# kenziyuliu/ChineseCheckersAgent

Measured on AMD Instinct MI355X. Metric: mcts_node_expansions_per_s (self-play with the policy/value net, 4096 games x 400 sims/move per GPU); BASELINE games/s = config.games_per_s: selfplay() calls that RETURNED per second, discarded ones included (train.py:61-64 counts them); config.games_won_per_s: those that returned a history, higher is better.
Workload: dtype f32

## Files before the change

### chinesecheckersagent_amd/csrc/ccsp_net.hip

```cpp
#include <cmath>
#include <cstring>
#include <type_traits>
#include <vector>
#include "ccsp_common.h"

namespace {

typedef float f32x4 __attribute__((ext_vector_type(4)));

#ifndef CCSP_NET_LDX
#define CCSP_NET_LDX 68
#define CCSP_NET_LDY 36
#endif
constexpr int LDX = CCSP_NET_LDX;
constexpr int LDY = CCSP_NET_LDY;
constexpr int LDI = 12;
constexpr int NPOL = 294, NPOL_PAD = 304;
#ifndef CCSP_NET_LDS_BIAS_ALL
#define CCSP_NET_LDS_BIAS_ALL 0
#endif
#ifndef CCSP_NET_PDG
#define CCSP_NET_PDG 1
#endif
#ifndef CCSP_NET_SEG_STEM
// ... 473 lines not shown
                  NW = C::NW, F32 = C::F32, F32A = C::F32A, F64 = C::F64, F64B = C::F64B, M64 = C::M64, XT = C::XT, HB = C::HB;
    constexpr bool AS = C::ALLSPLIT;
    extern __shared__ __attribute__((aligned(16))) unsigned char smem_raw[];
    Smem<C> &S = *reinterpret_cast<Smem<C> *>(smem_raw);
    const int tid = threadIdx.x, lane = tid & 63;
    const int wave = __builtin_amdgcn_readfirstlane(tid >> 6);
    const int q = lane >> 4, l15 = lane & 15;
    const long long s0 = (long long)blockIdx.x * NB;
    const int here = (int)((n - s0) < NB ? (n - s0) : NB);

    WBuf wb;
    wb.r = __builtin_amdgcn_make_buffer_rsrc(const_cast<float *>(W), 0, LAY.total * 4, 0x00020000);
    wb.voff = lane * 16;

#ifdef CCSP_STAMPS
    if (blockIdx.x == 0 && threadIdx.x == 0) net_stamps[62] = __builtin_amdgcn_s_memtime();
#endif
    float *in = S.y2;
    static_assert((PADROWS * LDY) % 4 == 0, "y1 is cleared 16 bytes at a time");
    for (int i = tid * 4; i < PADROWS * LDY; i += NTH * 4) *reinterpret_cast<f32x4 *>(&S.y1[i]) = f32x4{0.f, 0.f, 0.f, 0.f};
    if constexpr (NB < 8 || CCSP_NET_LDS_BIAS_ALL)
    for (int i = tid; i < BIAS_N / 4; i += NTH)
        *reinterpret_cast<f32x4 *>(&S.bias[4 * i]) = *reinterpret_cast<const f32x4 *>(W + LAY.trunk_b + 4 * i);
    const ccsp_request *rq = reinterpret_cast<const ccsp_request *>(planes) + s0;
    if constexpr (REQ) {
        static_assert((INROWS * LDI) % 4 == 0, "the staging area is cleared 16 bytes at a time");
        for (int i = tid * 4; i < INROWS * LDI; i += NTH * 4) *reinterpret_cast<f32x4 *>(&in[i]) = f32x4{0.f, 0.f, 0.f, 0.f};
        __syncthreads();
        struct PlaneWriter {
            float *base;
            struct Ref { float *p; __device__ __forceinline__ void operator=(uint8_t val) const { *p = (float)val; } };
            __device__ __forceinline__ Ref operator[](int i) const { const int cell = i / 7; return Ref{base + cell * LDI + (i - 7 * cell)}; }
        };
        for (int t = tid; t < here * 12; t += NTH) {
            const int s = t / 12, k = t - 12 * s;
            if (rq[s].kind == 0) continue;
            const ccsp_sr st = ccsp_load_sr(&rq[s].state);
            ccsp_scatter_checker(st, (int)rq[s].player, k, PlaneWriter{in + s * 49 * LDI});
        }
        for (int t = tid; t < here * 49; t += NTH) {
            const int s = t / 49, cell = t - 49 * s;
            if (rq[s].kind != 0 && rq[s].player == 2) in[(s * 49 + cell) * LDI + 6] = 1.0f;
        }
    } else if constexpr ((NB * 343) % 4 != 0) {
        for (int i = tid; i < INROWS * LDI; i += NTH) {
            const int cellg = i / LDI, ch = i % LDI, s = cellg / 49, cell = cellg % 49;
            in[i] = (ch < 7 && s < here) ? planes[(s0 + s) * 343 + cell * 7 + ch] : 0.0f;
        }
    } else {
        constexpr int NV = (NB * 343) / 4, PER = (NV + NTH - 1) / NTH;
        const f32x4 *src = reinterpret_cast<const f32x4 *>(planes + s0 * 343);
        const int nreal = here * 343;
        f32x4 v[PER];
#pragma unroll
        for (int r = 0; r < PER; r++) {
            const int e = (tid + r * NTH) * 4;
            v[r] = f32x4{0.f, 0.f, 0.f, 0.f};
            if (e + 3 < nreal) v[r] = src[tid + r * NTH];
            else if (e < nreal) { for (int j = 0; j < 4; j++) if (e + j < nreal) v[r][j] = planes[s0 * 343 + e + j]; }
        }
        static_assert((INROWS * LDI) % 4 == 0, "the staging area is cleared 16 bytes at a time");
        for (int i = tid * 4; i < INROWS * LDI; i += NTH * 4) *reinterpret_cast<f32x4 *>(&in[i]) = f32x4{0.f, 0.f, 0.f, 0.f};
        __syncthreads();
#pragma unroll
        for (int r = 0; r < PER; r++) {
            const int e = (tid + r * NTH) * 4;
#pragma unroll
            for (int j = 0; j < 4; j++) {
                const unsigned ee = (unsigned)(e + j);
                if ((int)ee < nreal) {
                    const unsigned cellg = __umulhi(ee, 613566757u);
                    in[cellg * LDI + (ee - 7u * cellg)] = v[r][j];
                }
            }
        }
    }
#ifdef CCSP_EXP_NET_INPUT_DELAY
    __builtin_amdgcn_s_sleep(CCSP_EXP_NET_INPUT_DELAY);
#endif
    __syncthreads();
    NET_STAMP(0);
#ifdef CCSP_STAMPS
    if (blockIdx.x == 0 && threadIdx.x == 0) net_stamps[60] = __builtin_amdgcn_s_memrealtime();
#endif

    const int nt2 = wave & 1, qr = wave >> 1, mt3 = AS ? qr % MT : F32 * qr;
    const int kshare = XT ? (C::CELLMAJOR ? (qr == 0 ? C::xseg_of(0) : (qr == 1 ? C::xseg_of(1) : (qr == 2 ? C::xseg_of(2) : C::xseg_of(3)))) : qr) : -1;
    const int kh = AS ? qr / MT : 0;
    f32x4 pre[NPREMAX];
    constexpr bool CM = C::CELLMAJOR;
    auto row_sp = [&](int row, int &s, int &pos) {
        if constexpr (CM) { const int t = row >> 4, l = row & 15; pos = cell_of<NB>(t < MT - 1 ? t * (16 / NB) + l / NB : 24); s = l % NB; }
        else { if (row >= ROWS) row -= 25; s = row / 25; pos = row % 25; }
    };
    auto y1_at = [&](int s, int pos, bool top_left) -> int {
        if constexpr (CM) return ((6 * (pos / 5) + pos % 5 + CM_PAD - (top_left ? 7 : 0)) * NB + s) * LDY + 4 * q;
        else return ((top_left ? 0 : PAD0) + s * PADPOS + (pos / 5) * 6 + (pos % 5)) * LDY + 4 * q;
    };
    constexpr int TAPROW = (CM ? NB : 1) * LDY;
    constexpr bool LDS_BIAS = NB < 8 || CCSP_NET_LDS_BIAS_ALL;
    auto bias4 = [&](int idx) -> f32x4 {
        if constexpr (LDS_BIAS) return *reinterpret_cast<const f32x4 *>(&S.bias[idx + 4 * q]);
        else return *reinterpret_cast<const f32x4 *>(W + LAY.trunk_b + idx + 4 * q);
    };
    auto relu4 = [](const f32x4 &v) -> f32x4 { return f32x4{relu(v[0]), relu(v[1]), relu(v[2]), relu(v[3])}; };

    f32x4 xr[F64];
    lds_float *const xown = lds_opaque(&S.x[(((wave >> 2) * M64) * 16 + l15) * LDX + (wave & 3) * 16 + 4 * q]);
    {
        const int nt = wave & 3, mt0 = (wave >> 2) * M64;
        int sbase[F64];
#pragma unroll
        for (int i = 0; i < F64; i++) {
            const int row = (mt0 + i) * 16 + l15;
            int s = row / 25, pos = row % 25;
            if constexpr (CM) row_sp(row, s, pos);
            sbase[i] = (s * 49 + (pos / 5) * 7 + (pos % 5)) * LDI + (q & 1) * 4;
        }
        int tapoff[5];
#pragma unroll
        for (int kb = 0; kb < 5; kb++) {
            const int tap = kb * 2 + (q >> 1);
            tapoff[kb] = ((tap / 3) * 7 + tap % 3) * LDI;
        }
        auto afrag = [&](int, int kb, int i) -> f32x4 {
            return *reinterpret_cast<const f32x4 *>(&in[sbase[i] + tapoff[kb]]);
        };
        const f32x4 bv = bias4(BIAS_STEM + nt * 16);
        auto epi = [&](int, const f32x4 &acc, int i) {
            xr[i] = relu4(acc + bv);
            lds_store4(xown, i * 16 * LDX, xr[i]);
        };
        prefetch<5>(wb, LAY.stem_w, nt, pre);
        auto next = [&]() { prefetch<4>(wb, LAY.l1_w[0], nt2, pre); };
        if (F64B == F64 || (wave >> 2) == 0) gemm_tiles<F64, 5, CCSP_NET_SEG_STEM>(wb, LAY.stem_w, nt, mt0, pre, afrag, next, epi);
        else gemm_tiles<F64B, 5, CCSP_NET_SEG_STEM>(wb, LAY.stem_w, nt, mt0, pre, afrag, next, epi);
    }
    __syncthreads();
    NET_STAMP(1);

    const lds_float *y1p[F32A + 1];
    bool prow_ok[F32A];
#pragma unroll
    for (int i = 0; i < F32A + 1; i++) {
        int s, pos;
        row_sp((i < F32A ? mt3 + i : MT - 1) * 16 + l15, s, pos);
        y1p[i] = lds_opaque(&S.y1[y1_at(s, pos, true)]);
        if (i < F32A) prow_ok[i] = (mt3 + i) * 16 + l15 < ROWS;
    }
    constexpr int CELL0 = 7 * TAPROW;
    const lds_float *const xin = lds_opaque(&S.x[(mt3 * 16 + l15) * LDX + 4 * q]);
    const lds_float *const xinx = lds_opaque(&S.x[((MT - 1) * 16 + l15) * LDX + 4 * q]);
    lds_float *const y2w = lds_opaque(&S.y2[(mt3 * 16 + l15) * LDY + nt2 * 16 + 4 * q]);
    const lds_float *const y2r = lds_opaque(&S.y2[(((wave >> 2) * M64) * 16 + l15) * LDY + 4 * q]);
    lds_float *const partw = lds_opaque(&S.part[AS ? mt3 * 2 + nt2 : nt2][(AS ? kh : (XT ? kshare : 0)) * (C::NSEG / C::NSH)][lane * 4]);
    const lds_float *const partr = lds_opaque(&S.part[AS ? ((wave >> 2) * M64) * 2 : 0][0][lane * 4]);
    constexpr bool TAIL4 = NB == 8 && CM && XT == 1 && CCSP_NET_TAIL_4X4 != 0;
    static_assert(!TAIL4 || (C::NSEG == 4 && NSPLIT == 4), "one segment job on each of the waves 0 .. 3");
    const int trow = 4 * ((lane >> 2) & 1) + (lane & 3), tcol = 4 * (lane >> 3) + (lane & 3);
    WBuf wbt = wb;
    wbt.voff = ((tcol >> 4) * 18 * 256 + (tcol & 15) * 4) * 4;
    const lds_float *ytail = nullptr;
    lds_float *partt = nullptr;
    if constexpr (TAIL4) {
        constexpr int pos = CELL8[24];
        ytail = lds_opaque(&S.y1[((6 * (pos / 5) + pos % 5 + CM_PAD - 7) * NB + trow) * LDY]);
        partt = lds_opaque(&S.part[tcol >> 4][0][(16 * ((tcol >> 2) & 3) + 4 * ((lane >> 2) & 1)) * 4 + (tcol & 3)]);
    }

    f32x4 bq2[AS ? 18 / C::NSH : 1];
    for (int blk = 0; blk < 9; blk++) {
        const int wo = blk * BLK_STRIDE, bb = BIAS_BLK + blk * BIAS_PER_BLK;
        int n2o = nt2 * 16;
        asm volatile("" : "+s"(n2o));
        {
            auto afrag = [&](int, int kb, int i) -> f32x4 {
                return i < F32A ? lds_load4(xin, i * 16 * LDX + kb * 16) : lds_load4(xinx, kb * 16);
            };
            const f32x4 bv = bias4(bb + BIAS_L1 + nt2 * 16);
            auto epi = [&](int, const f32x4 &acc, int i) {
                const lds_float *at = i == 0 ? y1p[0] : (i == 1 ? y1p[F32A > 1 ? 1 : 0] : y1p[F32A > 2 ? 2 : 0]);
                if constexpr (C::PADFULL) {
                    if (!(i == 0 ? prow_ok[0] : (i == 1 ? prow_ok[F32A > 1 ? 1 : 0] : prow_ok[F32A > 2 ? 2 : 0]))) return;
                }
                lds_store4(const_cast<lds_float *>(at), CELL0 + n2o, relu4(acc + bv));
            };
            auto epix = [&](const f32x4 &acc) {
                if (l15 < ROWS - (MT - 1) * 16) lds_store4(const_cast<lds_float *>(y1p[F32A]), CELL0 + n2o, relu4(acc + bv));
            };
            if constexpr (AS) ksplit_load<18, C::NSH>(wb, (LAY.l2_w[0] + wo), nt2, kh, bq2);
            if constexpr (AS) {
                auto epi1 = [&](int, const f32x4 &acc, int) {
                    if (prow_ok[0]) lds_store4(const_cast<lds_float *>(y1p[0]), CELL0 + n2o, relu4(acc + bv));
                };
                if (kh == 0) gemm_tiles<1, 4, CCSP_NET_SEG_L1>(wb, (LAY.l1_w[0] + wo), nt2, mt3, pre, afrag, []() {}, epi1);
            } else
            {
                auto next = [&]() { prefetch<18>(wb, (LAY.l2_w[0] + wo), nt2, pre); };
                if constexpr (CM && NB < 8) {
                    if (kshare == NSPLIT - 1) gemm_tiles_last<F32A, 4, NSPLIT, CCSP_NET_SEG_L1, 1>(wb, (LAY.l1_w[0] + wo), nt2, mt3, MT - 1, kshare, pre, afrag, next, epi, epix);
                    else gemm_tiles_last<F32A, 4, NSPLIT, CCSP_NET_SEG_L1, 0>(wb, (LAY.l1_w[0] + wo), nt2, mt3, MT - 1, kshare, pre, afrag, next, epi, epix);
                } else
                    gemm_tiles_last<F32A, 4, NSPLIT, CCSP_NET_SEG_L1, -1>(wb, (LAY.l1_w[0] + wo), nt2, mt3, MT - 1, kshare, pre, afrag, next, epi, epix);
            }
        }
        __syncthreads();
        NET_STAMP(2 + 3 * blk);
        {
            auto afrag = [&](int, int kb, int i) -> f32x4 {
                const int tap = kb >> 1;
                return lds_load4(y1p[i], ((tap / 3) * 6 + tap % 3) * TAPROW + (kb & 1) * 16);
            };
            const f32x4 bv = bias4(bb + BIAS_L2 + nt2 * 16);
            auto epi = [&](int, const f32x4 &acc, int i) { lds_store4(y2w, i * 16 * LDY, relu4(acc + bv)); };
            if constexpr (AS) {
                auto afrag_rt = [&](int kb) -> f32x4 {
                    const int tap = kb >> 1;
                    return lds_load4(y1p[0], ((tap / 3) * 6 + tap % 3) * TAPROW + (kb & 1) * 16);
                };
                gemm_ksplit<18, C::NSEG, C::NSH>(bq2, kh, afrag_rt, partw);
                prefetch<2>(wb, (LAY.l3_w[0] + wo), wave & 3, pre);
            } else
            {
                auto next = [&]() { prefetch<2>(wb, (LAY.l3_w[0] + wo), wave & 3, pre); };
                if constexpr (CM) {
                    auto run = [&](auto G) {
                        constexpr int g = decltype(G)::value;
                        if constexpr (TAIL4) {
                            gemm_tiles_split<F32A, 18, C::NSEG, NSPLIT, C::NE, true, C::dead_of(g, 0), C::dead_of(g, 1), -1>(wb, (LAY.l2_w[0] + wo), nt2, mt3, MT - 1, 0, pre, afrag, next, epi, partw);
                            if constexpr (g < 2) {
                                auto afrag4 = [&](int kb, int q4) -> f32x4 {
                                    const int tap = kb >> 1;
                                    return lds_load4(ytail, ((tap / 3) * 6 + tap % 3) * TAPROW + (kb & 1) * 16 + 4 * q4);
                                };
                                auto job = [&](auto SEG) {
                                    constexpr int seg = decltype(SEG)::value, kb0 = (18 * seg) / C::NSEG, kb1 = (18 * (seg + 1)) / C::NSEG;
                                    const f32x4 t = tail_tile_4x4<kb0, kb1 - kb0>(wbt, (LAY.l2_w[0] + wo), afrag4);
#pragma unroll
                                    for (int r = 0; r < 4; r++) partt[seg * 256 + r * 4] = t[r];
                                };
                                if (nt2 == 0) job(std::integral_constant<int, 2 * g>{});
                                else job(std::integral_constant<int, 2 * g + 1>{});
                            }
                        } else
                        gemm_tiles_split<F32A, 18, C::NSEG, NSPLIT, C::NE, true, C::dead_of(g, 0), C::dead_of(g, 1), C::xseg_of(g)>(wb, (LAY.l2_w[0] + wo), nt2, mt3, MT - 1, 0, pre, afrag, next, epi, partw);
                    };
                    if (qr == 0) run(std::integral_constant<int, 0>{});
                    else if (NSPLIT == 2 || qr == 1) run(std::integral_constant<int, 1>{});
                    else if (qr == 2) run(std::integral_constant<int, NSPLIT == 2 ? 1 : 2>{});
                    else run(std::integral_constant<int, NSPLIT == 2 ? 1 : 3>{});
                } else
                    gemm_tiles_split<F32A, 18, C::NSEG, NSPLIT, 0, false, 0u, 0u, 0>(wb, (LAY.l2_w[0] + wo), nt2, mt3, MT - 1, kshare, pre, afrag, next, epi, partw);
            }
            NET_STAMP(32 + blk);
#ifdef CCSP_STAMPS
            if (blockIdx.x == 0 && lane == 0 && blk == 4) {
                net_stamps[44 + wave] = __builtin_amdgcn_s_memtime();
                net_stamps[52 + wave] = __builtin_amdgcn_s_getreg(4 | (0 << 6) | (31 << 11));
            }
#endif
        }
        __syncthreads();
        NET_STAMP(3 + 3 * blk);
        {
            const int nt = wave & 3, half = wave >> 2, mt0 = half * M64;
            NET_STAMP2(0);
            const bool has_x = AS || (XT && half == C::NH - 1);
            constexpr int XSLOT = F64B - 1;
            const int xt = AS ? mt0 : 0;
            f32x4 ax[2];
            if (has_x) {
#pragma unroll
                for (int kb = 0; kb < 2; kb++) {
                    f32x4 v = lds_load4(partr, kb * C::NSEG * 256);
#pragma unroll
                    for (int c = 1; c < C::NSEG; c++) v = v + lds_load4(partr, (kb * C::NSEG + c) * 256);
                    ax[kb] = relu4(v + bias4(bb + BIAS_L2 + kb * 16));
                }
            }
            auto afrag = [&](int mt, int kb, int i) -> f32x4 {
                if (i == XSLOT && has_x) return ax[kb];
                return lds_load4(y2r, i * 16 * LDY + kb * 16);
            };
            const f32x4 bv = bias4(bb + BIAS_L3 + nt * 16);
            auto epi = [&](int mt, const f32x4 &acc, int i) {
                xr[i] = relu4(acc + bv + xr[i]);
                lds_store4(xown, i * 16 * LDX, xr[i]);
            };
            NET_STAMP2(1);
            auto next = [&]() {
                NET_STAMP2(2);
                prefetch<4>(wb, blk < 8 ? LAY.l1_w[0] + wo + BLK_STRIDE : LAY.pc_w, blk < 8 ? nt2 : 0, pre);
            };
            if (F64B == F64 || half == 0) gemm_tiles<F64, 2, CCSP_NET_SEG_L3>(wb, (LAY.l3_w[0] + wo), nt, mt0, pre, afrag, next, epi);
            else gemm_tiles<F64B, 2, CCSP_NET_SEG_L3>(wb, (LAY.l3_w[0] + wo), nt, mt0, pre, afrag, next, epi);
            NET_STAMP2(3);
        }
        __syncthreads();
        NET_STAMP2(4);
        NET_STAMP(4 + 3 * blk);
    }

    float *pc = S.y1;
    {
        const int mt0 = 2 * wave < MT - 2 ? 2 * wave : MT - 2;
        const lds_float *const xpc = lds_opaque(&S.x[(mt0 * 16 + l15) * LDX + 4 * q]);
        auto afrag = [&](int, int kb, int i) -> f32x4 { return lds_load4(xpc, i * 16 * LDX + kb * 16); };
        const f32x4 bv = bias4(BIAS_PC);
        int pcat[2];
#pragma unroll
        for (int i = 0; i < 2; i++) {
            const int row = (mt0 + i) * 16 + l15;
            int s, pos;
            row_sp(row, s, pos);
            pcat[i] = (CM ? (row < ROWS ? s * 25 + pos : row) : row) * 16 + 4 * q;
        }
        auto epi = [&](int, const f32x4 &acc, int i) {
            *reinterpret_cast<f32x4 *>(&pc[pcat[i]]) = relu4(acc + bv);
        };
        gemm_tiles<2, 4, CCSP_NET_SEG_PC>(wb, LAY.pc_w, 0, mt0, pre, afrag, []() {}, epi);
    }
    float *vc = S.y2;
    float *lg = S.y2 + 256;
    if (tid < ROWS) {
        const float *wv = W + LAY.vc_w;
        float acc = W[LAY.vc_b];
        const float *xr = &S.x[tid * LDX];
#pragma unroll 8
        for (int k = 0; k < 64; k++) acc += xr[k] * wv[k];
        int s, pos;
        row_sp(tid, s, pos);
        vc[CM ? s * 25 + pos : tid] = acc > 0.f ? acc : 0.f;
    }
    __syncthreads();
    NET_STAMP(29);

    float *part = S.x;
    {
        constexpr int GPQ = 25, NHALF = NW / 4, TPW = (5 + NHALF - 1) / NHALF, PG = HB / 4, PDG = C::PDG;
        const int kq = wave & 3, th = wave >> 2;
        int woff[TPW];
        bool valid[TPW];
#pragma unroll
        for (int t = 0; t < TPW; t++) {
            const int T = th * TPW + t;
            valid[t] = T < 5;
            woff[t] = LAY.pf_w + ((valid[t] ? T : 0) * 100 + kq * GPQ) * 256;
        }
        f32x4 acc[TPW][PG], bq[PDG + 1][TPW];
#pragma unroll
        for (int t = 0; t < TPW; t++)
#pragma unroll
            for (int g = 0; g < PG; g++) acc[t][g] = f32x4{0.f, 0.f, 0.f, 0.f};
#pragma unroll
        for (int d = 0; d < PDG; d++)
#pragma unroll
            for (int t = 0; t < TPW; t++) bq[d][t] = wb.load(woff[t] + d * 256);
        const float *arow = &pc[(lane & 3) * 400 + kq * GPQ * 4];
        f32x4 a[2][PG];
#pragma unroll
        for (int g = 0; g < PG; g++) a[0][g] = *reinterpret_cast<const f32x4 *>(arow + g * 1600);
#pragma unroll
        for (int kg = 0; kg < GPQ; kg++) {
            if (kg + 1 < GPQ) {
#pragma unroll
                for (int g = 0; g < PG; g++) a[(kg + 1) & 1][g] = *reinterpret_cast<const f32x4 *>(arow + g * 1600 + (kg + 1) * 4);
            }
            if (kg + PDG < GPQ) {
#pragma unroll
                for (int t = 0; t < TPW; t++) bq[(kg + PDG) % (PDG + 1)][t] = wb.load(woff[t] + (kg + PDG) * 256);
            }
#pragma unroll
            for (int t = 0; t < TPW; t++) {
                if (t + 1 < TPW || valid[t]) {
#pragma unroll
                    for (int j = 0; j < 4; j++)
#pragma unroll
                        for (int g = 0; g < PG; g++)
                            acc[t][g] = __builtin_amdgcn_mfma_f32_4x4x1f32(a[kg & 1][g][j], bq[kg % (PDG + 1)][t][j], acc[t][g], 0, 0, 0);
                }
            }
        }
#pragma unroll
        for (int t = 0; t < TPW; t++) {
            if (valid[t]) {
                const int T = th * TPW + t;
#pragma unroll
                for (int g = 0; g < PG; g++)
#pragma unroll
                    for (int r = 0; r < 4; r++) part[(kq * HB + 4 * g + r) * 320 + T * 64 + lane] = acc[t][g][r];
            }
        }
    }
    __syncthreads();
    for (int i = tid; i < NB * NPOL; i += NTH) {
        const int s = i / NPOL, col = i - s * NPOL;
        const float q0 = part[(0 * HB + s) * 320 + col], q1 = part[(1 * HB + s) * 320 + col], q2 = part[(2 * HB + s) * 320 + col],
                    q3 = part[(3 * HB + s) * 320 + col];
        lg[s * NPOL_PAD + col] = ((q0 + q1) + q2) + q3 + W[LAY.pf_b + col];
    }
    float *h1 = S.y2 + 256 + NB * NPOL_PAD;
    if (tid < NB * 32) {
        const int s = tid >> 5, u = tid & 31;
        const float *w1 = W + LAY.f1_w;
        float acc = W[LAY.f1_b + u];
#pragma unroll 5
        for (int i = 0; i < 25; i++) acc += vc[s * 25 + i] * w1[i * 32 + u];
        h1[s * 32 + u] = acc > 0.f ? acc : 0.f;
    }
    __syncthreads();
    NET_STAMP(30);
    if (tid < here) {
        const float *w2 = W + LAY.f2_w;
        float acc = W[LAY.f2_b];
        for (int u = 0; u < 32; u++) acc += h1[tid * 32 + u] * w2[u];
        if (!REQ || rq[tid].kind != 0) v_out[s0 + tid] = tanhf(acc);
    }
    for (int s = wave; s < here; s += NTH / 64) {
        const float *row = lg + s * NPOL_PAD;
        float mx = -INFINITY;
        for (int i = lane; i < NPOL; i += 64) mx = fmaxf(mx, row[i]);
        for (int m = 32; m >= 1; m >>= 1) mx = fmaxf(mx, __shfl_xor(mx, m));
        double e[5];
        double sum = 0.0;
#pragma unroll
        for (int j = 0; j < 5; j++) {
            const int i = lane + 64 * j;
            e[j] = i < NPOL ? exp((double)row[i] - (double)mx) : 0.0;
            sum += e[j];
        }
        for (int m = 32; m >= 1; m >>= 1) sum += __shfl_xor(sum, m);
        if constexpr (REQ) {
            double *pd = reinterpret_cast<double *>(S.x) + wave * 296;
            if (rq[s].kind != 0) {
#pragma unroll
                for (int j = 0; j < 5; j++) {
                    const int i = lane + 64 * j;
                    if (i < NPOL) pd[i] = e[j] / sum;
                }
                __builtin_amdgcn_wave_barrier();
                const int k = (int)rq[s].k < CCSP_MAX_MOVES ? (int)rq[s].k : CCSP_MAX_MOVES;
                const uint16_t *mrow = moves + (s0 + s) * CCSP_REQUEST_MOVES;
#pragma unroll
                for (int h = 0; h < 2; h++) {
                    const int j = lane + 64 * h;
                    if (j < k) { const int a = mrow[j] & 0x1FF; p_out[(s0 + s) * CCSP_REQUEST_MOVES + j] = a < NPOL ? pd[a] : 0.0; }
                }
                __builtin_amdgcn_wave_barrier();
            }
        } else {
#pragma unroll
        for (int j = 0; j < 5; j++) {
            const int i = lane + 64 * j;
            if (i < NPOL) {
                if (p_out) p_out[(s0 + s) * NPOL + i] = e[j] / sum;
                if (logits_out) logits_out[(s0 + s) * NPOL + i] = row[i];
            }
        }
        }
    }
    NET_STAMP(31);
#ifdef CCSP_STAMPS
    if (blockIdx.x == 0 && threadIdx.x == 0) net_stamps[61] = __builtin_amdgcn_s_memrealtime();
#endif
}

void pack_gemm(const std::vector<float> &Wkn, int K, int N, int KB, int NT, float *out) {
    for (int nt = 0; nt < NT; nt++)
        for (int kb = 0; kb < KB; kb++)
            for (int lane = 0; lane < 64; lane++)
                for (int j = 0; j < 4; j++) {
                    const int k = 16 * kb + 4 * (lane >> 4) + j, nn = 16 * nt + (lane & 15);
                    out[((nt * KB + kb) * 64 + lane) * 4 + j] = (k < K && nn < N) ? Wkn[(size_t)k * N + nn] : 0.0f;
                }
}

}

template <typename C, bool REQ = false>
static int launch_net(const float *packed, const float *planes, int n, float *logits, double *p, float *v, void *stream, bool *attr_set,
                      const uint16_t *moves = nullptr) {
    int dev = 0;
    CCSP_HIPCHK(hipGetDevice(&dev));
    if (dev < 0 || dev >= 64 || !attr_set[dev]) {
        CCSP_HIPCHK(hipFuncSetAttribute(reinterpret_cast<const void *>(net_forward_kernel<C, REQ>),
                                        hipFuncAttributeMaxDynamicSharedMemorySize, (int)sizeof(Smem<C>)));
        if (dev >= 0 && dev < 64) attr_set[dev] = true;
    }
    const int grid = (n + C::NB - 1) / C::NB;
    hipLaunchKernelGGL((net_forward_kernel<C, REQ>), dim3(grid), dim3(C::NTH), sizeof(Smem<C>), (hipStream_t)stream, packed, planes, n, logits, p, v, moves);
    CCSP_HIPCHK(hipGetLastError());
    return CCSP_OK;
}

static int g_net_shape = 0;
#ifndef CCSP_NET_SMALL
#define CCSP_NET_SMALL 1024
#define CCSP_NET_TINY 512
#endif
#ifndef CCSP_NET_ONE
#define CCSP_NET_ONE 256
#endif
static int pick_shape(int n) { return n <= CCSP_NET_ONE ? 1 : (n <= CCSP_NET_TINY ? 2 : (n <= CCSP_NET_SMALL ? 4 : 8)); }

extern "C" {

int ccsp_net_plain_size(void) { return PLAIN_TOTAL; }
int ccsp_net_packed_size(void) { return LAY.total; }

int ccsp_net_pack(const float *plain, float *packed) {
    if (!plain || !packed) return CCSP_EINVAL;
    memset(packed, 0, sizeof(float) * (size_t)LAY.total);
    const float *p = plain;
    {
        std::vector<float> Wkn(80 * 64, 0.0f);
        for (int tap = 0; tap < 9; tap++)
            for (int ch = 0; ch < 7; ch++)
                for (int o = 0; o < 64; o++) Wkn[(size_t)(tap * 8 + ch) * 64 + o] = p[(tap * 7 + ch) * 64 + o];
        pack_gemm(Wkn, 80, 64, 5, 4, packed + LAY.stem_w);
        p += 4032;
        memcpy(packed + LAY.stem_b, p, 64 * sizeof(float)); p += 64;
    }
    for (int b = 0; b < 9; b++) {
        { std::vector<float> Wkn(p, p + 64 * 32); pack_gemm(Wkn, 64, 32, 4, 2, packed + LAY.l1_w[b]); p += 2048; }
        memcpy(packed + LAY.l1_b[b], p, 32 * sizeof(float)); p += 32;
        { std::vector<float> Wkn(p, p + 288 * 32); pack_gemm(Wkn, 288, 32, 18, 2, packed + LAY.l2_w[b]); p += 9216; }
        memcpy(packed + LAY.l2_b[b], p, 32 * sizeof(float)); p += 32;
        { std::vector<float> Wkn(p, p + 32 * 64); pack_gemm(Wkn, 32, 64, 2, 4, packed + LAY.l3_w[b]); p += 2048; }
        memcpy(packed + LAY.l3_b[b], p, 64 * sizeof(float)); p += 64;
    }
    { std::vector<float> Wkn(p, p + 64 * 16); pack_gemm(Wkn, 64, 16, 4, 1, packed + LAY.pc_w); p += 1024; }
    memcpy(packed + LAY.pc_b, p, 16 * sizeof(float)); p += 16;
    for (int T = 0; T < 5; T++)
        for (int g = 0; g < 100; g++)
            for (int lane = 0; lane < 64; lane++)
                for (int j = 0; j < 4; j++) {
                    const int k = 4 * g + j, col = 64 * T + lane;
                    packed[LAY.pf_w + ((T * 100 + g) * 64 + lane) * 4 + j] = col < 294 ? p[(size_t)k * 294 + col] : 0.0f;
                }
    p += 117600;
    memcpy(packed + LAY.pf_b, p, 294 * sizeof(float)); p += 294;
    memcpy(packed + LAY.vc_w, p, 64 * sizeof(float)); p += 64;
    packed[LAY.vc_b] = *p; p += 1;
    memcpy(packed + LAY.f1_w, p, 800 * sizeof(float)); p += 800;
    memcpy(packed + LAY.f1_b, p, 32 * sizeof(float)); p += 32;
    memcpy(packed + LAY.f2_w, p, 32 * sizeof(float)); p += 32;
    packed[LAY.f2_b] = *p; p += 1;
    return (p - plain) == PLAIN_TOTAL ? CCSP_OK : CCSP_EINVAL;
}

int ccsp_debug_net_shape(int positions_per_workgroup) {
    g_net_shape = (positions_per_workgroup == 1 || positions_per_workgroup == 2 || positions_per_workgroup == 4 || positions_per_workgroup == 8) ? positions_per_workgroup : 0;
    return g_net_shape;
}

int ccsp_net_forward(const float *packed, const float *planes, int n, float *logits, double *p, float *v, void *stream) {
    if (n < 0 || (n > 0 && (!packed || !planes || !v))) return CCSP_EINVAL;
    if (n == 0) return CCSP_OK;
    static bool attr8[64] = {false}, attr4[64] = {false}, attr2[64] = {false}, attr1[64] = {false};
    const int shape = g_net_shape ? g_net_shape : pick_shape(n);
    if (shape == 1) return launch_net<Cfg<1, 8>>(packed, planes, n, logits, p, v, stream, attr1);
    if (shape == 2) return launch_net<Cfg<2, 8>>(packed, planes, n, logits, p, v, stream, attr2);
    if (shape == 4) return launch_net<Cfg<4, 4>>(packed, planes, n, logits, p, v, stream, attr4);
    return launch_net<Cfg<8, 8>>(packed, planes, n, logits, p, v, stream, attr8);
}

int ccsp_net_forward_requests(const float *packed, const ccsp_request *req, const uint16_t *moves, int n, double *pk, float *v, void *stream) {
    if (n < 0 || (n > 0 && (!packed || !req || !moves || !pk || !v))) return CCSP_EINVAL;
    if (n == 0) return CCSP_OK;
    static bool attr8[64] = {false}, attr4[64] = {false}, attr2[64] = {false}, attr1[64] = {false};
    const float *in = reinterpret_cast<const float *>(req);
    const int shape = g_net_shape ? g_net_shape : pick_shape(n);
    if (shape == 1) return launch_net<Cfg<1, 8>, true>(packed, in, n, nullptr, pk, v, stream, attr1, moves);
    if (shape == 2) return launch_net<Cfg<2, 8>, true>(packed, in, n, nullptr, pk, v, stream, attr2, moves);
    if (shape == 4) return launch_net<Cfg<4, 4>, true>(packed, in, n, nullptr, pk, v, stream, attr4, moves);
    return launch_net<Cfg<8, 8>, true>(packed, in, n, nullptr, pk, v, stream, attr8, moves);
}

#ifdef CCSP_STAMPS
int ccsp_debug_net_stamps(unsigned long long *out) {
    const bool more = out[63] == 0x5eedULL;
    CCSP_HIPCHK(hipMemcpyFromSymbol(out, HIP_SYMBOL(net_stamps), 64 * sizeof(unsigned long long)));
    if (more) CCSP_HIPCHK(hipMemcpyFromSymbol(out + 64, HIP_SYMBOL(net_stamps2), 64 * sizeof(unsigned long long)));
    return CCSP_OK;
}
#endif

}
```

Baseline: 23.12 million.

## Prefetch head weights and request data during policy-conv GEMM, stage into LDS

Hoists global loads for the policy bias, value FC1 weights/bias, value FC2 weights, and per-request kind/k/move indices into registers. These loads are issued inside the policy-conv GEMM's prefetch hook so their latency overlaps MFMA work. The head weights are then staged into the shared partial buffer and read from LDS. The value-conv dot product moves to the last waves with vectorized LDS loads, and FC2 weights are broadcast with readlane. This trades extra register pressure and more complex lane mapping for less serialized global-memory latency in the network tail.

Result: no change. 23.29 million (median of 6 runs) (+0.8%).

```diff
diff --git a/chinesecheckersagent_amd/csrc/ccsp_net.hip b/chinesecheckersagent_amd/csrc/ccsp_net.hip
--- a/chinesecheckersagent_amd/csrc/ccsp_net.hip
+++ b/chinesecheckersagent_amd/csrc/ccsp_net.hip
@@ -799,6 +799,53 @@
     }
 
     float *pc = S.y1;
+    float *vc = S.y2;
+    float *lg = S.y2 + 256;
+    constexpr int HW0 = LAY.pf_b, HWN = (LAY.f1_b + 32 - LAY.pf_b) / 4, HWR = (HWN + NTH - 1) / NTH;
+    static_assert(LAY.pf_b < LAY.f1_w && LAY.f1_w < LAY.f1_b && LAY.pf_b % 4 == 0 && (LAY.f1_b + 32 - LAY.pf_b) % 4 == 0 &&
+                  HWN * 4 <= 2 * C::XTILES * C::NSEG * 256, "pf_b .. f1_b: one 16-byte aligned run that fits Smem::part");
+    float *hw = &S.part[0][0][0];
+    const float *lgbias = hw, *f1w = hw + (LAY.f1_w - HW0), *f1b = hw + (LAY.f1_b - HW0);
+    f32x4 hwv[HWR];
+    constexpr int VD0 = NTH - NB * 32;
+    static_assert(LAY.f2_b == LAY.f2_w + 32 && NB <= NW, "the value output's bias follows its weights; a wave has at most one softmax position");
+    float f2l = 0.f;
+    unsigned vo_kind = 1, sm_kind = 1, sm_k = 0;
+    unsigned short sm_mv[2] = {0, 0};
+    auto heads_requests = [&]() {
+#pragma unroll
+        for (int r = 0; r < HWR; r++) {
+            const int t = tid + r * NTH;
+            hwv[r] = *reinterpret_cast<const f32x4 *>(W + HW0 + 4 * (t < HWN ? t : 0));
+        }
+        f2l = W[LAY.f2_w + (lane < 32 ? lane : 32)];
+        if constexpr (REQ) {
+            const int ss = (tid >> 6) < here ? (tid >> 6) : here - 1, sv = lane < here ? lane : here - 1;
+            vo_kind = rq[sv].kind;
+            sm_kind = rq[ss].kind;
+            sm_k = rq[ss].k;
+            const uint16_t *mrow = moves + (s0 + ss) * CCSP_REQUEST_MOVES;
+            sm_mv[0] = mrow[lane];
+            sm_mv[1] = mrow[lane + 64];
+        }
+    };
+    constexpr int VCW = (ROWS + 63) / 64, VC0 = (NW - VCW) * 64;
+    if (wave >= NW - VCW) {
+        const int row = tid - VC0;
+        if (row < ROWS) {
+            const float *wv = W + LAY.vc_w;
+            float acc = W[LAY.vc_b];
+            const lds_float *const xrow = lds_opaque(&S.x[row * LDX]);
+            f32x4 xv[16];
+#pragma unroll
+            for (int k4 = 0; k4 < 16; k4++) xv[k4] = lds_load4(xrow, 4 * k4);
+#pragma unroll
+            for (int k = 0; k < 64; k++) acc += xv[k >> 2][k & 3] * wv[k];
+            int s, pos;
+            row_sp(row, s, pos);
+            vc[CM ? s * 25 + pos : row] = acc > 0.f ? acc : 0.f;
+        }
+    }
     {
         const int mt0 = 2 * wave < MT - 2 ? 2 * wave : MT - 2;
         const lds_float *const xpc = lds_opaque(&S.x[(mt0 * 16 + l15) * LDX + 4 * q]);
@@ -815,19 +862,7 @@
         auto epi = [&](int, const f32x4 &acc, int i) {
             *reinterpret_cast<f32x4 *>(&pc[pcat[i]]) = relu4(acc + bv);
         };
-        gemm_tiles<2, 4, CCSP_NET_SEG_PC>(wb, LAY.pc_w, 0, mt0, pre, afrag, []() {}, epi);
-    }
-    float *vc = S.y2;
-    float *lg = S.y2 + 256;
-    if (tid < ROWS) {
-        const float *wv = W + LAY.vc_w;
-        float acc = W[LAY.vc_b];
-        const float *xr = &S.x[tid * LDX];
-#pragma unroll 8
-        for (int k = 0; k < 64; k++) acc += xr[k] * wv[k];
-        int s, pos;
-        row_sp(tid, s, pos);
-        vc[CM ? s * 25 + pos : tid] = acc > 0.f ? acc : 0.f;
+        gemm_tiles<2, 4, CCSP_NET_SEG_PC>(wb, LAY.pc_w, 0, mt0, pre, afrag, heads_requests, epi);
     }
     __syncthreads();
     NET_STAMP(29);
@@ -889,29 +924,38 @@
             }
         }
     }
+#pragma unroll
+    for (int r = 0; r < HWR; r++) {
+        const int t = tid + r * NTH;
+        if (t < HWN) *reinterpret_cast<f32x4 *>(&hw[4 * t]) = hwv[r];
+    }
     __syncthreads();
     for (int i = tid; i < NB * NPOL; i += NTH) {
         const int s = i / NPOL, col = i - s * NPOL;
         const float q0 = part[(0 * HB + s) * 320 + col], q1 = part[(1 * HB + s) * 320 + col], q2 = part[(2 * HB + s) * 320 + col],
                     q3 = part[(3 * HB + s) * 320 + col];
-        lg[s * NPOL_PAD + col] = ((q0 + q1) + q2) + q3 + W[LAY.pf_b + col];
+        lg[s * NPOL_PAD + col] = ((q0 + q1) + q2) + q3 + lgbias[col];
     }
     float *h1 = S.y2 + 256 + NB * NPOL_PAD;
-    if (tid < NB * 32) {
-        const int s = tid >> 5, u = tid & 31;
-        const float *w1 = W + LAY.f1_w;
-        float acc = W[LAY.f1_b + u];
-#pragma unroll 5
-        for (int i = 0; i < 25; i++) acc += vc[s * 25 + i] * w1[i * 32 + u];
+    if (tid >= VD0) {
+        const int s = (tid - VD0) >> 5, u = tid & 31;
+        float acc = f1b[u];
+#pragma unroll
+        for (int i = 0; i < 25; i++) acc += vc[s * 25 + i] * f1w[i * 32 + u];
         h1[s * 32 + u] = acc > 0.f ? acc : 0.f;
     }
     __syncthreads();
     NET_STAMP(30);
-    if (tid < here) {
-        const float *w2 = W + LAY.f2_w;
-        float acc = W[LAY.f2_b];
-        for (int u = 0; u < 32; u++) acc += h1[tid * 32 + u] * w2[u];
-        if (!REQ || rq[tid].kind != 0) v_out[s0 + tid] = tanhf(acc);
+    if (wave == NW - 1) {
+        float w2[33];
+#pragma unroll
+        for (int u = 0; u < 33; u++) w2[u] = __builtin_bit_cast(float, __builtin_amdgcn_readlane(__builtin_bit_cast(int, f2l), u));
+        if (lane < here) {
+            float acc = w2[32];
+#pragma unroll
+            for (int u = 0; u < 32; u++) acc += h1[lane * 32 + u] * w2[u];
+            if (!REQ || vo_kind != 0) v_out[s0 + lane] = tanhf(acc);
+        }
     }
     for (int s = wave; s < here; s += NTH / 64) {
         const float *row = lg + s * NPOL_PAD;
@@ -929,19 +973,18 @@
         for (int m = 32; m >= 1; m >>= 1) sum += __shfl_xor(sum, m);
         if constexpr (REQ) {
             double *pd = reinterpret_cast<double *>(S.x) + wave * 296;
-            if (rq[s].kind != 0) {
+            if (sm_kind != 0) {
 #pragma unroll
                 for (int j = 0; j < 5; j++) {
                     const int i = lane + 64 * j;
                     if (i < NPOL) pd[i] = e[j] / sum;
                 }
                 __builtin_amdgcn_wave_barrier();
-                const int k = (int)rq[s].k < CCSP_MAX_MOVES ? (int)rq[s].k : CCSP_MAX_MOVES;
-                const uint16_t *mrow = moves + (s0 + s) * CCSP_REQUEST_MOVES;
+                const int k = (int)sm_k < CCSP_MAX_MOVES ? (int)sm_k : CCSP_MAX_MOVES;
 #pragma unroll
                 for (int h = 0; h < 2; h++) {
                     const int j = lane + 64 * h;
-                    if (j < k) { const int a = mrow[j] & 0x1FF; p_out[(s0 + s) * CCSP_REQUEST_MOVES + j] = a < NPOL ? pd[a] : 0.0; }
+                    if (j < k) { const int a = sm_mv[h] & 0x1FF; p_out[(s0 + s) * CCSP_REQUEST_MOVES + j] = a < NPOL ? pd[a] : 0.0; }
                 }
                 __builtin_amdgcn_wave_barrier();
             }
```
